# lancedb/lance

Hardware: AMD Instinct MI355X
Metric: QPS @ recall@10 (SIFT-1M IVF_PQ nlist=256 M=16) + index-build sec (higher is better)
Workload: dtype f32; 1 GPU; SIFT-1M-like 1Mx128 f32, IVF_PQ nlist=256 M=16 nbits=8, build+search on MI355X; n=1000000, d=128, nlist=256, m=16, k=10, nprobes=10, refine_factor=10, parallelism=single

## Files before the change

lance_amd/csrc/build.hip:

```cpp
#include <vector>

#include <hip/hip_fp16.h>

#include "common.h"
#include "exact.cuh"
#include <cstdlib>

#include "index.h"
#include "kernels.h"

#pragma clang fp contract(off)

namespace lh {

template <bool F16>
__global__ __launch_bounds__(256) void normalize_kernel(const float *__restrict__ x, int64_t n, int d, float *__restrict__ out) {
  const int64_t r = (int64_t)blockIdx.x * 256 + threadIdx.x;
  if (r >= n) return;
  const float *v = x + r * d;
  float acc = 0.0f;
  for (int i = 0; i < d; ++i) {
    float p = v[i] * v[i];
    if (F16) p = __half2float(__float2half_rn(p));
    acc = acc + p;
// ... 210 lines not shown
  return LANCE_HIP_OK;
}

}

using namespace lh;

lance_hip_index::~lance_hip_index() {
  (void)hipSetDevice(device);
  if (centroids) (void)hipFree(centroids);
  if (codebook) (void)hipFree(codebook);
  if (cb_mean) (void)hipFree(cb_mean);
  if (pt) {
    if (pt->g) (void)hipFree(pt->g);
    if (pt->cen_t) (void)hipFree(pt->cen_t);
    if (pt->row_beta) (void)hipFree(pt->row_beta);
    if (pt->beta_min) (void)hipFree(pt->beta_min);
    if (pt->beta_abs) (void)hipFree(pt->beta_abs);
    if (pt->beta_mean) (void)hipFree(pt->beta_mean);
    delete pt;
  }
  if (cq) {
    if (cq->cpl) (void)hipFree(cq->cpl);
    if (cq->maxbits) (void)hipFree(cq->maxbits);
    delete cq;
  }
  if (ms) {
    if (ms->cbh) (void)hipFree(ms->cbh);
    if (ms->cbn2) (void)hipFree(ms->cbn2);
    if (ms->row_cn2) (void)hipFree(ms->row_cn2);
    if (ms->cmaxp) (void)hipFree(ms->cmaxp);
    delete ms;
  }
  if (part_offsets) (void)hipFree(part_offsets);
  if (codes) (void)hipFree(codes);
  if (row_ids) (void)hipFree(row_ids);
  if (vectors) (void)hipFree(vectors);
  if (flat_items) (void)hipFree(flat_items);
  if (raw_u8) (void)hipFree(raw_u8);
  if (rq_rot_t) (void)hipFree(rq_rot_t);
}

static int encode_finish(lance_hip_ctx *ctx, uint64_t n, uint32_t nlist, const float *dists, const uint32_t *part_ids, double *loss_out_host) {
  LH_CHECK_HIP(hipGetLastError());
  if (loss_out_host) {
    std::vector<float> dh(n);
// ... 324 lines not shown
```

lance_amd/csrc/index.h:

```cpp
#pragma once
#include <atomic>
#include <cstdint>
#include <mutex>
#include <vector>

struct int2_host { int x, y; };

inline uint64_t lance_hip_next_index_serial() {
  static std::atomic<uint64_t> next{1};
  return next.fetch_add(1, std::memory_order_relaxed);
}

struct lance_hip_index {
  uint64_t serial = lance_hip_next_index_serial();
  bool ephemeral = false;
  int device = 0;
  int metric = 0;
  int dtype = 0;
  uint32_t d = 0, nlist = 0, m = 0, nbits = 8;
  uint64_t n = 0;
  float *centroids = nullptr;
  float *codebook = nullptr;
  bool model_finite = true;
  float *cb_mean = nullptr;
  struct PtConst {
    float *g = nullptr;
    float *cen_t = nullptr;
    float *row_beta = nullptr;
    float *beta_min = nullptr;
    float *beta_abs = nullptr;
    float *beta_mean = nullptr;
  } *pt = nullptr;
  struct MsConst {
    bool usable = false;
    float sigma = 1.0f;
    void *cbh = nullptr;
    float *cbn2 = nullptr;
    float *row_cn2 = nullptr;
    float cmax = 0.0f;
    float cmax_full = 0.0f;
    float *cmaxp = nullptr;
    uint32_t sum_rs = 0, max_rs = 0;
  } *ms = nullptr;
  struct CqConst {
    uint16_t *cpl = nullptr;
    uint32_t *maxbits = nullptr;
  } *cq = nullptr;
  std::mutex lazy_mu;
  uint32_t *part_offsets = nullptr;
  std::vector<uint32_t> part_offsets_h;
  uint8_t *codes = nullptr;
  uint64_t *row_ids = nullptr;
  int2_host *flat_items = nullptr;
  uint32_t n_flat_items = 0;
  float *vectors = nullptr;
  const void *raw = nullptr;
  uint64_t n_raw = 0;
  uint8_t *raw_u8 = nullptr;
  uint64_t raw_gen = 0;
  int raw_compact_state = 0;
  bool sq = false;
  double sq_lo = 0.0, sq_hi = 0.0;
  uint32_t sq_nlist = 0, sq_ld = 0;
  const uint32_t *sq_xx = nullptr;
  bool rq = false;
  uint32_t rq_nlist = 0, rq_cb = 0;
  float *rq_rot_t = nullptr;
  const float *rq_add = nullptr;
// ... 6 lines not shown
```

lance_amd/csrc/kernels.h:

```cpp
#pragma once
#include <stdint.h>

#include "common.h"
#include "search_plan.h"

namespace lh {

struct PairwiseArgs {
  const void *x_native = nullptr;
  int x_dtype = 0;
  const float *x = nullptr;
  bool lanes32 = false;
  int64_t n = 0;
  int64_t ldx = 0;
  int x_batch_off = 0;
  const float *cent = nullptr;
  int k = 0;
  int64_t cent_batch_stride = 0;
  const float *bias = nullptr;
  int64_t bias_batch_stride = 0;
  uint32_t *ids = nullptr;
  float *dists = nullptr;
  int64_t out_batch_stride = 0;
  uint8_t *codes = nullptr;
// ... 97 lines not shown
int widen_into(lance_hip_ctx *ctx, int dtype, const void *p, size_t count, float *dst);
int from_f32(lance_hip_ctx *ctx, int dtype, const float *src, void *dst, size_t count);
int launch_residual(lance_hip_ctx *ctx, const float *x, int64_t n, int d, const float *cent, const uint32_t *part_ids, float *out, bool f16);


int ivfpq_scan_merge_pm(lance_hip_ctx *ctx, const lance_hip_index *ix, const IvfpqPlan &plan, const float *qs, uint32_t nq, const uint32_t *probes,
                        uint32_t nprobes, uint32_t keff, uint32_t k, bool do_refine, uint64_t *ids, float *dists,
                        uint64_t *cand_rid, uint32_t *cand_cnt, uint32_t *flags, const uint32_t *allow);
int find_partitions_f32(lance_hip_ctx *ctx, int metric, const float *qf, uint32_t nq, uint32_t d, const float *cf, uint32_t nlist,
                        uint32_t nprobes, uint32_t *part_ids, float *dists, bool lanes32);
struct PairLists {
  const uint64_t *row_ids;
  int nprobes, k;
  uint32_t *pkey, *ppos;
  uint32_t *pcnt, *pamb;
  uint32_t *flags;
  uint32_t *n_replay;
};
int sq_merge_pairs(lance_hip_ctx *ctx, const PairLists &pl, uint32_t nq, uint64_t *ids, float *dists, const char *timer);
bool flat_small_supported(int metric, int dtype, uint32_t d, uint32_t nq, uint32_t k, uint64_t n);
int flat_topk_small(lance_hip_ctx *ctx, int metric, int dtype, const void *x, const uint64_t *row_ids, uint64_t n, uint32_t d, const float *q,
                    uint32_t nq, uint32_t k, uint64_t *ids, float *dists, bool *done);
bool coarse_mfma_supported(int metric, int d, uint32_t nq, uint32_t nlist, uint32_t nprobes, bool lanes32, const float *q, const float *cent);
int find_partitions_mfma(lance_hip_ctx *ctx, int metric, const float *q, uint32_t nq, int d, const float *cent, uint32_t nlist, uint32_t nprobes,
                         float *matrix, uint32_t *part_ids, float *dists, const uint16_t *cpl_ready = nullptr, const uint32_t *maxbits_ready = nullptr);
int launch_normalize(lance_hip_ctx *ctx, const float *x, int64_t n, int d, float *out, bool f16);
int launch_normalize_planes(lance_hip_ctx *ctx, const float *x, int64_t n, int d, float *out, bool f16, uint16_t *plane16, int dp, float *n2);

int qscan_index_constants(lance_hip_ctx *ctx, lance_hip_index *ix);
int index_alloc_like_pq(lance_hip_ctx *ctx, const lance_hip_index *src, lance_hip_index **out);
constexpr int QSCAN_SEG_CAP = 256;
struct SelectOut;
int qscan_classb_to_rescan(lance_hip_ctx *ctx, const uint32_t *tbound, uint32_t nq, uint32_t nprobes, uint32_t *seg_cnt, uint32_t *qovf);
int qscan_nearest_keys(lance_hip_ctx *ctx, const uint32_t *probes, uint32_t nq, uint32_t nprobes, uint32_t *keys, uint32_t nb = 1);
int qscan_group(lance_hip_ctx *ctx, const uint32_t *probes, uint32_t nq, uint32_t nprobes, int nlist, const uint32_t *tglobal,
                uint32_t *keys, uint32_t *tbound, uint32_t *pair_starts, uint32_t *pair_idx, uint32_t *item_start4, int4 *desc4,
                uint32_t max_items4, int G = 4, int dot = 0);
int qbound_launch(lance_hip_ctx *ctx, const lance_hip_index *ix, const float *qs, uint32_t nq, uint32_t keff, const uint32_t *pair_starts0,
                  const uint32_t *pair_idx0, uint32_t *item_start, int4 *desc, uint32_t max_items, uint32_t *tglobal, const uint32_t *allow);
int qscan_launch(lance_hip_ctx *ctx, const lance_hip_index *ix, const float *qs, uint32_t nq, uint32_t nprobes, const uint32_t *pair_idx,
                 const uint32_t *item_start4, const int4 *desc4, uint32_t max_items4, const uint32_t *tbound, uint32_t *seg_cnt,
                 uint32_t *seg_pos, uint32_t *qovf, const uint32_t *allow, const uint32_t *probes, const IvfpqPlan &plan);
int qbound_pt_launch(lance_hip_ctx *ctx, const lance_hip_index *ix, const float *qs, uint32_t nq, uint32_t nprobes, uint32_t keff,
                     const uint32_t *probes, const uint32_t *pair_starts0, const uint32_t *pair_idx0, uint32_t *item_start, int4 *desc,
                     uint32_t max_items, uint32_t *tglobal, const uint32_t *allow);
int qmerge_launch(lance_hip_ctx *ctx, const lance_hip_index *ix, const float *qs, uint32_t nq, const uint32_t *probes, uint32_t nprobes,
                  const uint32_t *tbound, uint32_t *tglobal, const uint32_t *seg_cnt, const uint32_t *seg_pos, const uint32_t *qovf,
                  uint32_t *pool_key, uint32_t *pool_pos, uint32_t *pool_cnt, int pool_cap, const SelectOut &o, const uint32_t *allow,
// ... 15 lines not shown
```

lance_amd/csrc/mfma_assign.hip:

```cpp
#include <algorithm>
#include <cstdlib>
#include <cstring>

#include <hip/hip_fp16.h>

#include "common.h"
#include "exact.cuh"
#include "kernels.h"
#include "ma_common.cuh"

#pragma clang fp contract(off)

namespace lh {

__global__ __launch_bounds__(64) void ma_prep_kernel(const float *__restrict__ cent, int k, int d, int dp, const float *__restrict__ bias,
                                                     uint16_t *__restrict__ chi, uint16_t *__restrict__ clo, float *__restrict__ cn,
                                                     uint32_t *__restrict__ maxbits ,
                                                     const uint8_t *__restrict__ active) {
  if (active && !active[0]) return;
  const int c = blockIdx.x;
  float s = 0.0f;
  for (int e = threadIdx.x; e < dp; e += 64) {
    const float v = e < d ? cent[(int64_t)c * d + e] : 0.0f;
    const uint32_t hb = bf16_rne_bits(v);
// ... 1021 lines not shown
      for (int dd = k2 >> 1; dd > 0; dd >>= 1) {
        if (dd >= 64) {
          const unsigned long long a = v2[0], b = v2[1];
          if (a > b) { v2[0] = b; v2[1] = a; }
        } else {
#pragma unroll
          for (int jr = 0; jr < 2; ++jr) {
            const int e = jr * 64 + lane;
            const unsigned long long o = __shfl_xor(v2[jr], dd, 64);
            const bool up = (e & k2) == 0, lower = (lane & dd) == 0;
            v2[jr] = (lower == up) ? (v2[jr] < o ? v2[jr] : o) : (v2[jr] > o ? v2[jr] : o);
          }
        }
      }
    }
    if (base + 64 >= cnt) break;
  }
  if (lane < nprobes) {
    part_ids[(int64_t)qi * nprobes + lane] = (uint32_t)v2[0];
    if (dists) dists[(int64_t)qi * nprobes + lane] = key_to_float((uint32_t)(v2[0] >> 32));
  }
}

bool coarse_mfma_supported(int metric, int d, uint32_t nq, uint32_t nlist, uint32_t nprobes, bool lanes32, const float *q, const float *cent) {
  static const char *env = getenv("LANCE_HIP_MFMA_COARSE");
  static const bool off = env && env[0] == '0', force = env && env[0] == '1';
  if (off || lanes32 || (metric != METRIC_L2 && metric != METRIC_DOT)) return false;
  if (nprobes == 0 || nprobes > 64 || nprobes > nlist) return false;
  if ((reinterpret_cast<uintptr_t>(q) | reinterpret_cast<uintptr_t>(cent)) & 15) return false;
  if (d <= 128) { if (d % 16 != 0 || d < 16 || nlist < 32) return false; }
  else if (d > 4096 || nlist < 64 || d % 4 != 0) return false;
  if (force) return true;
  if (d > 128) return (uint64_t)nq * nlist >= (1ull << 23);
  return (uint64_t)nq * nlist * (uint64_t)d >= (1ull << 27);
}

template <int KS>
static void coarse_launch_narrow(lance_hip_ctx *ctx, const MaArgs &a, int metric, dim3 grid) {
  constexpr int D = KS * 16;
  const size_t lds_x = (size_t)MA_ROWS * (D + 4) * 4;
  const size_t lds_c = (size_t)2 * 2 * MA_CT * (D + 8) * 2 + (size_t)2 * 2 * MA_CT * 4;
  const size_t lds = std::max(lds_x, lds_c);
  if (a.gkey) {
    if (metric == METRIC_DOT) hipLaunchKernelGGL((ma_top3_kernel<KS, METRIC_DOT, float, 2>), grid, dim3(256), lds, ctx->stream, a);
    else hipLaunchKernelGGL((ma_top3_kernel<KS, METRIC_L2, float, 2>), grid, dim3(256), lds, ctx->stream, a);
    return;
  }
  if (metric == METRIC_DOT) hipLaunchKernelGGL((ma_top3_kernel<KS, METRIC_DOT, float, 1>), grid, dim3(256), lds, ctx->stream, a);
  else hipLaunchKernelGGL((ma_top3_kernel<KS, METRIC_L2, float, 1>), grid, dim3(256), lds, ctx->stream, a);
}

static int coarse_groups_from() {
  static const int v = getenv("LANCE_HIP_COARSE_GROUPS") ? atoi(getenv("LANCE_HIP_COARSE_GROUPS")) : 1024;
  return v;
}
bool coarse_groups_shape(int d, uint32_t nlist) {
  static const bool ma = getenv("LANCE_HIP_COARSE_GROUPS_MA") != nullptr;
  return !ma && d <= 128 && d % 16 == 0 && coarse_groups_from() > 0 && nlist >= (uint32_t)std::max(coarse_groups_from(), 256);
}

int find_partitions_mfma(lance_hip_ctx *ctx, int metric, const float *q, uint32_t nq, int d, const float *cent, uint32_t nlist, uint32_t nprobes,
                         float *matrix, uint32_t *part_ids, float *dists, const uint16_t *cpl_ready, const uint32_t *maxbits_ready) {
  const bool wide = d > 128;
  const int dp = wide ? (d + MW_KC - 1) / MW_KC * MW_KC : d;
  const size_t kd = (size_t)nlist * dp;
  uint16_t *chi = ctx->scratch_t<uint16_t>("cq.chi", kd), *clo = ctx->scratch_t<uint16_t>("cq.clo", kd);
  float *cn = ctx->scratch_t<float>("cq.cn", (size_t)nlist);
  uint32_t *maxbits = ctx->scratch_t<uint32_t>("cq.maxbits", 4);
  float *e2 = ctx->scratch_t<float>("cq.e2", (size_t)nq);
  if (!chi || !clo || !cn || !maxbits || !e2) return LANCE_HIP_ENOMEM;
  const int groups_from = coarse_groups_from();
  const bool groups = !wide && groups_from > 0 && nlist >= (uint32_t)std::max(groups_from, 256);
  const int ng = groups ? (int)cdiv(nlist, MA_CT) * 4 : 0;
  float *gkey = nullptr, *gsec = nullptr;
  if (groups) {
    gkey = ctx->scratch_t<float>("cq.gkey", (size_t)nq * 2 * ng);
    gsec = gkey;
    if (!gkey) return LANCE_HIP_ENOMEM;
  }
  LH_CHECK_HIP(lh::memset_async(maxbits, 0, 16, ctx->stream));
  static const bool groups_ma = getenv("LANCE_HIP_COARSE_GROUPS_MA") != nullptr;
  if (groups && !groups_ma) {
    ScopedTimer t(ctx, "dist_matrix");
    LH_TRY(launch_xform_sweep_groups(ctx, metric, q, nq, d, cent, nlist, maxbits, gkey, ng, e2, cpl_ready, maxbits_ready));
  } else {
// ... 69 lines not shown
```

lance_amd/csrc/search.hip:

```cpp
#include <algorithm>
#include <cstdlib>
#include <string>
#include <vector>

#include "common.h"
#include "exact.cuh"
#include "index.h"
#include "kernels.h"
#include "search_common.cuh"

#pragma clang fp contract(off)

namespace lh {

#ifndef LH_SCAN_CAP
#define LH_SCAN_CAP 1024
#endif
#ifndef LH_SCAN_ROUND
#define LH_SCAN_ROUND 512
#endif
#ifndef LH_LUT_BATCH
#define LH_LUT_BATCH 4
#endif
constexpr int SCAN_CAP = LH_SCAN_CAP;
// ... 880 lines not shown
      const f4 v = x[i * 4 + p];
      uint32_t pk = 0;
#pragma unroll
      for (int e = 0; e < 4; ++e) {
        const uint32_t b = (v[e] >= 0.0f && v[e] < 256.0f) ? (uint32_t)v[e] : 0u;
        ok = ok && (float)b == v[e];
        pk |= b << (8 * e);
      }
      w[p] = pk;
    }
    out[i] = make_uint4(w[0], w[1], w[2], w[3]);
  }
  if (__any(!ok) && (threadIdx.x & 63) == 0) atomicOr(bad, 1u);
}

static bool raw_compact_enabled() {
  static const bool off = getenv("LANCE_HIP_NO_RAW_COMPACT") != nullptr;
  return !off;
}
int coarse_planes_prepare(lance_hip_ctx *ctx, const lance_hip_index *ix_c, int scan_metric) {
  lance_hip_index *ix = const_cast<lance_hip_index *>(ix_c);
  std::lock_guard<std::mutex> lk(ix->lazy_mu);
  if (ix->cq || ctx->capturing) return LANCE_HIP_OK;
  auto *cq = new lance_hip_index::CqConst();
  bool ok = hipMalloc(reinterpret_cast<void **>(&cq->cpl), xform_coarse_planes_elems(ix->nlist, (int)ix->d) * 2) == hipSuccess;
  ok = ok && hipMalloc(reinterpret_cast<void **>(&cq->maxbits), 16) == hipSuccess;
  auto drop = [&]() { if (cq->cpl) (void)hipFree(cq->cpl); if (cq->maxbits) (void)hipFree(cq->maxbits); delete cq; };
  if (!ok) { (void)hipGetLastError(); drop(); return LANCE_HIP_OK; }
  if (lh::memset_async(cq->maxbits, 0, 16, ctx->stream) != hipSuccess ||
      xform_coarse_planes(ctx, scan_metric, ix->centroids, ix->nlist, (int)ix->d, cq->cpl, cq->maxbits) != LANCE_HIP_OK ||
      hipStreamSynchronize(ctx->stream) != hipSuccess) {
    drop();
    set_error("find_partitions: building the centroid planes of the index failed");
    return LANCE_HIP_ERUNTIME;
  }
  ix->cq = cq;
  return LANCE_HIP_OK;
}

const uint8_t *raw_compact_prepare(lance_hip_ctx *ctx, const lance_hip_index *ix_c) {
  lance_hip_index *ix = const_cast<lance_hip_index *>(ix_c);
  if (!raw_compact_enabled() || ix->dtype != LANCE_HIP_F32 || !ix->raw || ix->n_raw == 0 || (ix->d & 15) != 0 ||
      (ix->metric != LANCE_HIP_L2 && ix->metric != LANCE_HIP_DOT) || (reinterpret_cast<uintptr_t>(ix->raw) & 15) != 0)
    return nullptr;
  std::lock_guard<std::mutex> lk(ix->lazy_mu);
  if (ix->raw_compact_state != 0) return ix->raw_compact_state > 0 ? ix->raw_u8 : nullptr;
  if (ctx->capturing) return nullptr;
  const uint64_t bytes = ix->n_raw * (uint64_t)ix->d;
  uint8_t *buf = nullptr;
  uint32_t *bad = ctx->scratch_t<uint32_t>("raw.compact_flag", 1);
  if (!bad || hipMalloc(reinterpret_cast<void **>(&buf), bytes) != hipSuccess) {
    (void)hipGetLastError();
    ix->raw_compact_state = -1;
// ... 406 lines not shown

  uint32_t *flags = ctx->scratch_t<uint32_t>("search.flags", (size_t)nq + 1);
  if (!flags) return LANCE_HIP_ENOMEM;
  LH_CHECK_HIP(lh::memset_async(flags, 0, ((size_t)nq + 1) * 4, ctx->stream));
  uint32_t *n_fallback = flags + nq;
  ctx->last_replay_counter = n_fallback;
  if (flags_out) *flags_out = flags;
  if (nq == 0) return LANCE_HIP_OK;

  float *qn = ix->metric == LANCE_HIP_COSINE ? ctx->scratch_t<float>("search.qnorm", (size_t)nq * d) : nullptr;
  if (ix->metric == LANCE_HIP_COSINE && !qn) return LANCE_HIP_ENOMEM;
  const float *qs = qn ? qn : q;
  PlanBatch pb;
  pb.nq = nq; pb.nprobes = nprobes; pb.keff = keff; pb.has_range = has_range != 0;
  IvfpqPlan plan = plan_ivfpq_search(plan_index(ix, qs), pb, plan_switches_from_env());
  if (plan.wants_ms_constants) {
    LH_REQUIRE(!ctx->capturing, "search: the index's matrix-core constants would have to be built during a graph capture");
    LH_TRY(mscan_prepare(ctx, const_cast<lance_hip_index *>(ix)));
    plan = plan_ivfpq_search(plan_index(ix, qs), pb, plan_switches_from_env());
  }
  static const bool q_stats = getenv("LANCE_HIP_Q_STATS") != nullptr;
  if (q_stats && plan.route != ROUTE_QUANTISED) fprintf(stderr, "[plan] nq=%u nprobes=%u keff=%u route %d: %s\n", nq, nprobes, keff, (int)plan.route, plan.why);
  if (qn) LH_TRY(launch_normalize(ctx, q, (int64_t)nq, d, qn, ix->dtype == LANCE_HIP_F16));
  float *matrix = ctx->scratch_t<float>("search.matrix", (size_t)nq * nlist);
  uint32_t *probes = ctx->scratch_t<uint32_t>("search.probes", (size_t)nq * nprobes);
  if (!matrix || !probes) return LANCE_HIP_ENOMEM;
  const bool coarse_l32 = ix->dtype == LANCE_HIP_F16 && scan_metric == LANCE_HIP_DOT && d > 16;
  if (coarse_mfma_supported(scan_metric, d, nq, (uint32_t)nlist, nprobes, coarse_l32, qs, ix->centroids)) {
    const uint16_t *cpl = nullptr;
    const uint32_t *cmb = nullptr;
    if (coarse_groups_shape(d, (uint32_t)nlist)) {
      LH_TRY(coarse_planes_prepare(ctx, ix, scan_metric));
      if (ix->cq) { cpl = ix->cq->cpl; cmb = ix->cq->maxbits; }
    }
    LH_TRY(find_partitions_mfma(ctx, scan_metric, qs, nq, d, ix->centroids, (uint32_t)nlist, nprobes, matrix, probes, nullptr, cpl, cmb));
  } else {
    PairwiseArgs pa;
    pa.x = qs; pa.n = nq; pa.ldx = d; pa.cent = ix->centroids; pa.k = nlist; pa.matrix = matrix;
    pa.lanes32 = coarse_l32;
    LH_TRY(launch_dist_matrix(ctx, pa, d, scan_metric, 1));
    ScopedTimer t(ctx, "select_probes");
    launch_select_probes(ctx, matrix, nlist, (int)nprobes, (int)nq, probes, nullptr);
  }
  uint64_t *cand_rid = nullptr;
  uint32_t *cand_cnt = nullptr;
  if (do_refine) {
    cand_rid = ctx->scratch_t<uint64_t>("search.cand_rid", (size_t)nq * keff);
    cand_cnt = ctx->scratch_t<uint32_t>("search.cand_cnt", nq);
    if (!cand_rid || !cand_cnt) return LANCE_HIP_ENOMEM;
  }
  const bool fast = plan.route != ROUTE_EXACT_ONLY;
  const bool use_pm = plan.route == ROUTE_PAIR_SCAN || plan.route == ROUTE_QUANTISED;
  int nsplit = 1;
  if (nq < (uint32_t)(2 * ctx->num_cus)) {
    nsplit = (int)std::min<uint64_t>({8ull, (uint64_t)nprobes, cdiv(2ull * ctx->num_cus, nq)});
    if (nsplit < 1) nsplit = 1;
  }
  const size_t nblk = (size_t)nq * nsplit;
// ... 61 lines not shown
    const int dpad = (d + 3) & ~3;
    const size_t lds = (size_t)dpad * 4 + (size_t)m * 256 * 4 + (size_t)keff * 12 + ((size_t)keff + 1) * 8 + 64 * 4 + 16 +
                       16 + (size_t)std::max<uint32_t>(200, keff) * 4 + (size_t)m * 16 + 16;
    LH_REQUIRE(lds <= 160 * 1024, "search: exact kernel does not fit in LDS (m=%d, k*refine=%u)", m, keff);
    ScopedTimer t(ctx, "ivfpq_exact");
    if (ix->nbits == 4) {
      if (scan_metric == LANCE_HIP_DOT) hipLaunchKernelGGL((ivfpq_exact_kernel<METRIC_DOT, 4>), dim3(nq), dim3(64), lds, ctx->stream, ea);
      else hipLaunchKernelGGL((ivfpq_exact_kernel<METRIC_L2, 4>), dim3(nq), dim3(64), lds, ctx->stream, ea);
    } else {
      if (scan_metric == LANCE_HIP_DOT) hipLaunchKernelGGL((ivfpq_exact_kernel<METRIC_DOT, 8>), dim3(nq), dim3(64), lds, ctx->stream, ea);
      else hipLaunchKernelGGL((ivfpq_exact_kernel<METRIC_L2, 8>), dim3(nq), dim3(64), lds, ctx->stream, ea);
    }
  }
  if (do_refine) LH_TRY(launch_refine(ctx, ix, q, nq, d, cand_rid, cand_cnt, keff, k, ids, dists, flags, nullptr));
  LH_CHECK_HIP(hipGetLastError());
  return LANCE_HIP_OK;
}

int find_partitions_f32(lance_hip_ctx *ctx, int metric, const float *qf, uint32_t nq, uint32_t d, const float *cf, uint32_t nlist,
                        uint32_t nprobes, uint32_t *part_ids, float *dists, bool lanes32) {
  if (nprobes > nlist) nprobes = nlist;
  LH_REQUIRE(nlist <= 8192 || nprobes <= 2048, "find_partitions: nprobes=%u > 2048 with more than 8192 partitions is not supported", nprobes);
  if (nq == 0 || nprobes == 0) return LANCE_HIP_OK;
  float *matrix = ctx->scratch_t<float>("search.matrix", (size_t)nq * nlist);
  if (!matrix) return LANCE_HIP_ENOMEM;
  const int km = metric == LANCE_HIP_COSINE ? LANCE_HIP_L2 : metric;
  if (coarse_mfma_supported(km, (int)d, nq, nlist, nprobes, lanes32, qf, cf)) {
    LH_TRY(find_partitions_mfma(ctx, km, qf, nq, (int)d, cf, nlist, nprobes, matrix, part_ids, dists));
  } else {
    PairwiseArgs pa;
    pa.x = qf; pa.n = nq; pa.ldx = d;
    pa.cent = cf; pa.k = (int)nlist; pa.matrix = matrix;
    pa.lanes32 = lanes32;
    LH_TRY(launch_dist_matrix(ctx, pa, (int)d, km, 1));
    launch_select_probes(ctx, matrix, (int)nlist, (int)nprobes, (int)nq, part_ids, dists);
  }
  LH_CHECK_HIP(hipGetLastError());
  LH_CHECK_HIP(hipStreamSynchronize(ctx->stream));
  return LANCE_HIP_OK;
}

static int check_flags(lance_hip_ctx *ctx, const uint32_t *flags, uint32_t nq) {
  std::vector<uint32_t> fh(nq);
  LH_CHECK_HIP(hipMemcpyAsync(fh.data(), flags, (size_t)nq * 4, hipMemcpyDeviceToHost, ctx->stream));
  LH_CHECK_HIP(hipStreamSynchronize(ctx->stream));
  uint32_t n_over = 0, n_amb = 0, n_bad = 0;
  for (uint32_t i = 0; i < nq; ++i) { n_over += (fh[i] & FLAG_OVERFLOW) ? 1 : 0; n_amb += (fh[i] & FLAG_AMBIGUOUS) ? 1 : 0; n_bad += (fh[i] & FLAG_BADROW) ? 1 : 0; }
  if (n_bad) {
    set_error("search: refine met row ids beyond the %s raw vectors given to lance_hip_index_set_raw (%u queries): the raw array must be "
              "indexed by the stored row ids", "attached", n_bad);
    return LANCE_HIP_EINVAL;
  }
  if (n_over || n_amb) {
    set_error("search: internal error, %u overflow / %u ambiguous queries were not resolved by the exact kernel", n_over, n_amb);
    return LANCE_HIP_ERUNTIME;
  }
  return LANCE_HIP_OK;
}

}

using namespace lh;

extern "C" {

int lance_hip_index_prewarm(lance_hip_ctx *ctx, lance_hip_index *idx) {
  lh::CtxLock _ctx_lock(ctx);
  LH_REQUIRE(ctx && idx, "index_prewarm: NULL argument");
  LH_CHECK_HIP(hipSetDevice(ctx->device));
  if (idx->m > 0 && !plan_index_ms_refusal(plan_index(idx, nullptr), plan_switches_from_env())) LH_TRY(mscan_prepare(ctx, idx));
  if (coarse_groups_shape((int)idx->d, idx->nlist) && (reinterpret_cast<uintptr_t>(idx->centroids) & 15) == 0)
    LH_TRY(coarse_planes_prepare(ctx, idx, idx->metric == LANCE_HIP_COSINE ? LANCE_HIP_L2 : idx->metric));
  (void)raw_compact_prepare(ctx, idx);
  LH_CHECK_HIP(hipStreamSynchronize(ctx->stream));
  return LANCE_HIP_OK;
}

int lance_hip_find_partitions(lance_hip_ctx *ctx, int dtype, int metric, const void *q, uint32_t nq, uint32_t d,
                              const void *centroids, uint32_t nlist, uint32_t nprobes, uint32_t *part_ids, float *dists) {
  lh::CtxLock _ctx_lock(ctx);
  LH_REQUIRE(ctx && q && centroids && part_ids, "find_partitions: NULL argument");
  LH_TRY(check_dtype(dtype, "find_partitions"));
  LH_REQUIRE(nlist > 0 && nlist <= 65536, "find_partitions: nlist=%u not supported in this version (1..65536)", nlist);
  LH_CHECK_HIP(hipSetDevice(ctx->device));
  const float *qf, *cf;
  LH_TRY(as_f32(ctx, dtype, q, (size_t)nq * d, "f16.q", &qf));
  LH_TRY(as_f32(ctx, model_dtype(dtype), centroids, (size_t)nlist * d, "f16.cent", &cf));
  return find_partitions_f32(ctx, metric, qf, nq, d, cf, nlist, nprobes, part_ids, dists, dtype == LANCE_HIP_F16 && metric == LANCE_HIP_DOT && d > 16);
}

int lance_hip_ivfpq_search_async(lance_hip_ctx *ctx, const lance_hip_index *idx, const void *q, uint32_t nq, uint32_t k,
                                 uint32_t nprobes, uint32_t refine_factor, uint64_t *ids, float *dists) {
  lh::CtxLock _ctx_lock(ctx);
  LH_REQUIRE(ctx && idx && (nq == 0 || (q && ids && dists)), "search: NULL argument");
// ... 166 lines not shown
```

Baseline: 25.38 million queries/s.

## Fuse coarse centroid distance GEMM with top-nprobes selection in one kernel

Adds a fused coarse-quantizer kernel. It computes query-centroid distances with split-bf16 MFMA (hi/lo planes) into LDS, then picks the probe candidates within an error bound, rescored exactly in fp32, all in the same kernel. This removes the nq x nlist distance matrix written to global memory and the separate select_probes launch. Centroid hi/lo planes and norms are precomputed and cached per index. Rows with too many or too few candidates, or NaN, fall back to an exact per-row scan, which adds complexity and can be slow when many rows take that path.

```diff
diff --git a/lance_amd/csrc/build.hip b/lance_amd/csrc/build.hip
--- a/lance_amd/csrc/build.hip
+++ b/lance_amd/csrc/build.hip
@@ -256,6 +256,7 @@
   }
   if (cq) {
     if (cq->cpl) (void)hipFree(cq->cpl);
+    if (cq->chi) (void)hipFree(cq->chi);
     if (cq->maxbits) (void)hipFree(cq->maxbits);
     delete cq;
   }
diff --git a/lance_amd/csrc/index.h b/lance_amd/csrc/index.h
--- a/lance_amd/csrc/index.h
+++ b/lance_amd/csrc/index.h
@@ -44,6 +44,8 @@
   } *ms = nullptr;
   struct CqConst {
     uint16_t *cpl = nullptr;
+    uint16_t *chi = nullptr, *clo = nullptr;
+    float *cn = nullptr;
     uint32_t *maxbits = nullptr;
   } *cq = nullptr;
   std::mutex lazy_mu;
diff --git a/lance_amd/csrc/kernels.h b/lance_amd/csrc/kernels.h
--- a/lance_amd/csrc/kernels.h
+++ b/lance_amd/csrc/kernels.h
@@ -143,8 +143,17 @@
 int flat_topk_small(lance_hip_ctx *ctx, int metric, int dtype, const void *x, const uint64_t *row_ids, uint64_t n, uint32_t d, const float *q,
                     uint32_t nq, uint32_t k, uint64_t *ids, float *dists, bool *done);
 bool coarse_mfma_supported(int metric, int d, uint32_t nq, uint32_t nlist, uint32_t nprobes, bool lanes32, const float *q, const float *cent);
+struct CoarseFusedConst {
+  const uint16_t *chi, *clo;
+  const float *cn;
+  const uint32_t *maxbits;
+};
+bool coarse_fused_shape(int d, uint32_t nlist);
+size_t coarse_fused_cn_elems(uint32_t nlist);
+int coarse_fused_planes(lance_hip_ctx *ctx, const float *cent, uint32_t nlist, int d, uint16_t *chi, uint16_t *clo, float *cn, uint32_t *maxbits );
 int find_partitions_mfma(lance_hip_ctx *ctx, int metric, const float *q, uint32_t nq, int d, const float *cent, uint32_t nlist, uint32_t nprobes,
-                         float *matrix, uint32_t *part_ids, float *dists, const uint16_t *cpl_ready = nullptr, const uint32_t *maxbits_ready = nullptr);
+                         float *matrix, uint32_t *part_ids, float *dists, const uint16_t *cpl_ready = nullptr, const uint32_t *maxbits_ready = nullptr,
+                         const CoarseFusedConst *fused_ready = nullptr);
 int launch_normalize(lance_hip_ctx *ctx, const float *x, int64_t n, int d, float *out, bool f16);
 int launch_normalize_planes(lance_hip_ctx *ctx, const float *x, int64_t n, int d, float *out, bool f16, uint16_t *plane16, int dp, float *n2);
 
diff --git a/lance_amd/csrc/mfma_assign.hip b/lance_amd/csrc/mfma_assign.hip
--- a/lance_amd/csrc/mfma_assign.hip
+++ b/lance_amd/csrc/mfma_assign.hip
@@ -1067,6 +1067,259 @@
   }
 }
 
+constexpr int CF_ROWS = 32;
+constexpr int CF_WAVES = 8;
+constexpr uint32_t CF_MAX_LISTS = 960;
+
+static size_t coarse_fused_lds(int d, uint32_t nlist) {
+  const size_t n64 = (size_t)cdiv(nlist, MA_CT) * MA_CT;
+  const size_t planes = (size_t)2 * CF_ROWS * (d + 8) * 2, cands = (size_t)CF_WAVES * CS_CAP * 12;
+  return (size_t)CF_ROWS * (d + 4) * 4 + std::max(planes, cands) + (size_t)CF_ROWS * (n64 + 4) * 4;
+}
+
+template <int CTRL, int ROW_MASK, bool SUM>
+__device__ __forceinline__ float cf_dpp_step(float v) {
+  const float ident = SUM ? 0.0f : v;
+  const float o = __builtin_bit_cast(float, __builtin_amdgcn_update_dpp(__builtin_bit_cast(int, ident), __builtin_bit_cast(int, v), CTRL, ROW_MASK, 0xF, false));
+  return SUM ? v + o : fminf(v, o);
+}
+template <bool SUM>
+__device__ __forceinline__ float cf_wave_reduce(float v) {
+  v = cf_dpp_step<0xB1, 0xF, SUM>(v);
+  v = cf_dpp_step<0x4E, 0xF, SUM>(v);
+  v = cf_dpp_step<0x141, 0xF, SUM>(v);
+  v = cf_dpp_step<0x140, 0xF, SUM>(v);
+  v = cf_dpp_step<0x142, 0xA, SUM>(v);
+  v = cf_dpp_step<0x143, 0xC, SUM>(v);
+  return __builtin_bit_cast(float, __builtin_amdgcn_readlane(__builtin_bit_cast(int, v), 63));
+}
+
+template <int KS, int METRIC>
+__global__ __launch_bounds__(64 * CF_WAVES, 4) void coarse_fused_kernel(const float *__restrict__ q, int nq, const uint16_t *__restrict__ chi,
+                                                                       const uint16_t *__restrict__ clo, const float *__restrict__ cn ,
+                                                                       const uint32_t *__restrict__ maxbits, const float *__restrict__ cent, int nlist,
+                                                                       int nprobes, uint32_t *__restrict__ part_ids, float *__restrict__ dists,
+                                                                       uint32_t *__restrict__ n_exact_rows) {
+  extern __shared__ __attribute__((aligned(16))) char smem[];
+  constexpr int D = KS * 16;
+  constexpr int XS = D + 4;
+  constexpr int CS = D + 8;
+  constexpr size_t PLANES = (size_t)2 * CF_ROWS * CS * 2, CANDS = (size_t)CF_WAVES * CS_CAP * 12;
+  const int n64 = (nlist + MA_CT - 1) / MA_CT * MA_CT;
+  const int SP = n64 + 4;
+  float *xs = reinterpret_cast<float *>(smem);
+  uint16_t *xh = reinterpret_cast<uint16_t *>(xs + CF_ROWS * XS), *xl = xh + CF_ROWS * CS;
+  unsigned long long *ck_all = reinterpret_cast<unsigned long long *>(xh);
+  uint32_t *cl_all = reinterpret_cast<uint32_t *>(ck_all + CF_WAVES * CS_CAP);
+  float *sur = reinterpret_cast<float *>(smem + (size_t)CF_ROWS * XS * 4 + (PLANES > CANDS ? PLANES : CANDS));
+  const int lane = threadIdx.x & 63, wave = threadIdx.x >> 6, grp = lane >> 4;
+  const int j = lane & 31, g = lane >> 5;
+  const int64_t row0 = (int64_t)blockIdx.x * CF_ROWS;
+
+  if ((int)threadIdx.x < CF_ROWS * (D / 8)) {
+    const int r = (int)threadIdx.x / (D / 8), c8 = (int)threadIdx.x - r * (D / 8);
+    f4 a = {0.0f, 0.0f, 0.0f, 0.0f}, b = a;
+    if (row0 + r < nq) { a = load4(q + (row0 + r) * D + 8 * c8); b = load4(q + (row0 + r) * D + 8 * c8 + 4); }
+    *reinterpret_cast<f4 *>(&xs[r * XS + 8 * c8]) = a;
+    *reinterpret_cast<f4 *>(&xs[r * XS + 8 * c8 + 4]) = b;
+    const float v[8] = {a.x, a.y, a.z, a.w, b.x, b.y, b.z, b.w};
+    bf16x8 h, l;
+#pragma unroll
+    for (int e = 0; e < 8; ++e) {
+      const uint32_t hb = bf16_rne_bits(v[e]);
+      const uint32_t lb = bf16_rne_bits(v[e] - bf16_bits_to_float(hb));
+      h[e] = (short)hb; l[e] = (short)lb;
+    }
+    *reinterpret_cast<bf16x8 *>(xh + r * CS + 8 * c8) = h;
+    *reinterpret_cast<bf16x8 *>(xl + r * CS + 8 * c8) = l;
+  }
+  __syncthreads();
+
+  const int nblocks = n64 / 32;
+  for (int blk = wave; blk < nblocks; blk += CF_WAVES) {
+    const int c0 = blk * 32;
+    const int ca = min(c0 + j, nlist - 1);
+    const uint16_t *ha = chi + (int64_t)ca * D + g * 8, *la = clo + (int64_t)ca * D + g * 8;
+    const uint16_t *bh = xh + j * CS + g * 8, *bl = xl + j * CS + g * 8;
+    bf16x8 ah[KS], al[KS];
+#pragma unroll
+    for (int s = 0; s < KS; ++s) {
+      ah[s] = *reinterpret_cast<const bf16x8 *>(ha + s * 16);
+      al[s] = *reinterpret_cast<const bf16x8 *>(la + s * 16);
+    }
+    f32x16 acc;
+#pragma unroll
+    for (int v = 0; v < 16; ++v) acc[v] = 0.0f;
+#pragma unroll
+    for (int s = 0; s < KS; ++s) {
+      const bf16x8 qh = *reinterpret_cast<const bf16x8 *>(bh + s * 16);
+      const bf16x8 ql = *reinterpret_cast<const bf16x8 *>(bl + s * 16);
+      acc = __builtin_amdgcn_mfma_f32_32x32x16_bf16(ah[s], qh, acc, 0, 0, 0);
+      acc = __builtin_amdgcn_mfma_f32_32x32x16_bf16(ah[s], ql, acc, 0, 0, 0);
+      acc = __builtin_amdgcn_mfma_f32_32x32x16_bf16(al[s], qh, acc, 0, 0, 0);
+    }
+    float *srow = sur + (size_t)j * SP;
+#pragma unroll
+    for (int vq = 0; vq < 4; ++vq) {
+      const int ib = c0 + 8 * vq + 4 * g;
+      const f4 cn4 = *reinterpret_cast<const f4 *>(cn + ib);
+      float o[4];
+#pragma unroll
+      for (int e = 0; e < 4; ++e) {
+        const float dot = acc[vq * 4 + e];
+        float v = METRIC == METRIC_DOT ? -dot : __builtin_fmaf(-2.0f, dot, cn4[e]);
+        if (ib + e >= nlist) v = INFINITY;
+        o[e] = v;
+      }
+      *reinterpret_cast<f4 *>(srow + ib) = f4{o[0], o[1], o[2], o[3]};
+    }
+  }
+  __syncthreads();
+
+  unsigned long long *ck = ck_all + wave * CS_CAP;
+  uint32_t *cl = cl_all + wave * CS_CAP;
+  const float cmax2 = __uint_as_float(maxbits[0]);
+  for (int r = wave; r < CF_ROWS; r += CF_WAVES) {
+    const int64_t qi = row0 + r;
+    if (qi >= nq) break;
+    float *row = sur + (size_t)r * SP;
+    const float *wrow = xs + r * XS;
+    float xn2 = 0.0f;
+    for (int e = lane; e < D; e += 64) xn2 += wrow[e] * wrow[e];
+    xn2 = cf_wave_reduce<true>(xn2);
+    const float E2 = 2.0f * 0.0001220703125f * (xn2 + cmax2) + (METRIC == METRIC_DOT ? 4.7683716e-7f : 0.0f);
+    bool bad = !(E2 < INFINITY) || !(E2 > 7.888609052210118e-31f);
+    float m0 = INFINITY, m1 = INFINITY, m2 = INFINITY, m3 = INFINITY;
+    for (int base = 0; base < n64; base += 256) {
+      float v4[4];
+#pragma unroll
+      for (int u = 0; u < 4; ++u) { const int i = base + 64 * u + lane; v4[u] = i < n64 ? row[i] : INFINITY; }
+#pragma unroll
+      for (int u = 0; u < 4; ++u) {
+        const float v = v4[u];
+        bad |= v != v;
+        if (v < m3) {
+          if (v < m2) {
+            m3 = m2;
+            if (v < m1) {
+              m2 = m1;
+              if (v < m0) { m1 = m0; m0 = v; } else m1 = v;
+            } else m2 = v;
+          } else m3 = v;
+        }
+      }
+    }
+    bad = __any(bad);
+    uint32_t cnt = 0;
+    if (!bad) {
+      float t0 = INFINITY;
+      for (int pr = 0; pr < nprobes; ++pr) {
+        t0 = cf_wave_reduce<false>(m0);
+        if (!(t0 < INFINITY)) break;
+        const unsigned long long holders = __ballot(m0 == t0);
+        if (lane == __ffsll((long long)holders) - 1) { m0 = m1; m1 = m2; m2 = m3; m3 = INFINITY; }
+      }
+      const float thr = t0 + E2;
+      for (int base = 0; base < nlist; base += 256) {
+        float v4[4];
+#pragma unroll
+        for (int u = 0; u < 4; ++u) { const int i = base + 64 * u + lane; v4[u] = i < nlist ? row[i] : INFINITY; }
+#pragma unroll
+        for (int u = 0; u < 4; ++u) {
+          const int i = base + 64 * u + lane;
+          const bool take = i < nlist && v4[u] <= thr;
+          const unsigned long long mask = __ballot(take);
+          if (take) {
+            const uint32_t pos = cnt + (uint32_t)__popcll(mask & ((1ull << lane) - 1ull));
+            if (pos < (uint32_t)CS_CAP) cl[pos] = (uint32_t)i;
+          }
+          cnt += (uint32_t)__popcll(mask);
+        }
+      }
+      if (cnt > (uint32_t)CS_CAP || cnt < (uint32_t)nprobes) bad = true;
+    }
+    __builtin_amdgcn_wave_barrier();
+    if (bad) {
+      if (lane == 0 && n_exact_rows) atomicAdd(n_exact_rows, 1u);
+      for (int c0 = 0; c0 < nlist; c0 += 4) {
+        const int c = c0 + grp;
+        float v = 0.0f;
+        if (c < nlist) v = cs_group_distance<METRIC>(wrow, cent + (int64_t)c * D, D, lane);
+        else (void)cs_group_distance<METRIC>(wrow, cent, D, lane);
+        if (c < nlist && (lane & 15) == 0) row[c] = v;
+      }
+      __builtin_amdgcn_wave_barrier();
+      __threadfence_block();
+      unsigned long long last = 0ull;
+      bool have_last = false;
+      for (int pr = 0; pr < nprobes; ++pr) {
+        unsigned long long best = ~0ull;
+        for (int i = lane; i < nlist; i += 64) {
+          const unsigned long long kk = ((unsigned long long)order_key(row[i]) << 32) | (uint32_t)i;
+          if ((!have_last || kk > last) && kk < best) best = kk;
+        }
+#pragma unroll
+        for (int o = 32; o > 0; o >>= 1) { const unsigned long long ob = __shfl_xor(best, o, 64); best = ob < best ? ob : best; }
+        if (lane == 0) {
+          part_ids[qi * nprobes + pr] = (uint32_t)best;
+          if (dists) dists[qi * nprobes + pr] = key_to_float((uint32_t)(best >> 32));
+        }
+        last = best; have_last = true;
+      }
+      continue;
+    }
+    for (uint32_t c0 = 0; c0 < cnt; c0 += 16) {
+      uint32_t cc[4];
+      float dv[4];
+#pragma unroll
+      for (int u = 0; u < 4; ++u) { const uint32_t ci = c0 + 4 * u + (uint32_t)grp; cc[u] = ci < cnt ? cl[ci] : cl[0]; }
+#pragma unroll
+      for (int u = 0; u < 4; ++u) dv[u] = cs_group_distance<METRIC>(wrow, cent + (int64_t)cc[u] * D, D, lane);
+#pragma unroll
+      for (int u = 0; u < 4; ++u) {
+        const uint32_t ci = c0 + 4 * u + (uint32_t)grp;
+        if (ci < cnt && (lane & 15) == 0) ck[ci] = ((unsigned long long)order_key(dv[u]) << 32) | cc[u];
+      }
+    }
+    __builtin_amdgcn_wave_barrier();
+    const unsigned long long k0 = (uint32_t)lane < cnt ? ck[lane] : ~0ull, k1 = 64u + (uint32_t)lane < cnt ? ck[64 + lane] : ~0ull;
+    uint32_t rank0 = 0, rank1 = 0;
+    for (uint32_t i = 0; i < cnt; i += 4) {
+      unsigned long long o[4];
+#pragma unroll
+      for (uint32_t u = 0; u < 4; ++u) o[u] = i + u < cnt ? ck[i + u] : ~0ull;
+#pragma unroll
+      for (uint32_t u = 0; u < 4; ++u) {
+        rank0 += o[u] < k0 ? 1u : 0u;
+        rank1 += o[u] < k1 ? 1u : 0u;
+      }
+    }
+    if ((uint32_t)lane < cnt && rank0 < (uint32_t)nprobes) {
+      part_ids[qi * nprobes + rank0] = (uint32_t)k0;
+      if (dists) dists[qi * nprobes + rank0] = key_to_float((uint32_t)(k0 >> 32));
+    }
+    if (64u + (uint32_t)lane < cnt && rank1 < (uint32_t)nprobes) {
+      part_ids[qi * nprobes + rank1] = (uint32_t)k1;
+      if (dists) dists[qi * nprobes + rank1] = key_to_float((uint32_t)(k1 >> 32));
+    }
+    __builtin_amdgcn_wave_barrier();
+  }
+}
+
+template <int KS>
+static void coarse_launch_fused(lance_hip_ctx *ctx, int metric, const float *q, uint32_t nq, const uint16_t *chi, const uint16_t *clo, const float *cn,
+                                const uint32_t *maxbits, const float *cent, uint32_t nlist, uint32_t nprobes, uint32_t *part_ids, float *dists,
+                                uint32_t *n_exact_rows) {
+  const size_t lds = coarse_fused_lds(KS * 16, nlist);
+  const dim3 grid((unsigned)cdiv(nq, CF_ROWS));
+  if (metric == METRIC_DOT)
+    hipLaunchKernelGGL((coarse_fused_kernel<KS, METRIC_DOT>), grid, dim3(64 * CF_WAVES), lds, ctx->stream, q, (int)nq, chi, clo, cn, maxbits, cent, (int)nlist,
+                       (int)nprobes, part_ids, dists, n_exact_rows);
+  else
+    hipLaunchKernelGGL((coarse_fused_kernel<KS, METRIC_L2>), grid, dim3(64 * CF_WAVES), lds, ctx->stream, q, (int)nq, chi, clo, cn, maxbits, cent, (int)nlist,
+                       (int)nprobes, part_ids, dists, n_exact_rows);
+}
+
 bool coarse_mfma_supported(int metric, int d, uint32_t nq, uint32_t nlist, uint32_t nprobes, bool lanes32, const float *q, const float *cent) {
   static const char *env = getenv("LANCE_HIP_MFMA_COARSE");
   static const bool off = env && env[0] == '0', force = env && env[0] == '1';
@@ -1104,8 +1357,66 @@
   return !ma && d <= 128 && d % 16 == 0 && coarse_groups_from() > 0 && nlist >= (uint32_t)std::max(coarse_groups_from(), 256);
 }
 
+bool coarse_fused_shape(int d, uint32_t nlist) {
+  static const bool off = getenv("LANCE_HIP_NO_COARSE_FUSED") != nullptr && getenv("LANCE_HIP_NO_COARSE_FUSED")[0] == '1';
+  return !off && d >= 16 && d <= 128 && d % 16 == 0 && nlist >= 32 && nlist <= CF_MAX_LISTS && !coarse_groups_shape(d, nlist) &&
+         coarse_fused_lds(d, nlist) <= (size_t)160 * 1024;
+}
+size_t coarse_fused_cn_elems(uint32_t nlist) { return (size_t)cdiv(nlist, MA_CT) * MA_CT; }
+int coarse_fused_planes(lance_hip_ctx *ctx, const float *cent, uint32_t nlist, int d, uint16_t *chi, uint16_t *clo, float *cn, uint32_t *maxbits) {
+  hipLaunchKernelGGL(ma_prep_kernel, dim3(nlist), dim3(64), 0, ctx->stream, cent, (int)nlist, d, d, nullptr, chi, clo, cn, maxbits, nullptr);
+  LH_CHECK_HIP(hipGetLastError());
+  return LANCE_HIP_OK;
+}
+
+static int find_partitions_fused(lance_hip_ctx *ctx, int metric, const float *q, uint32_t nq, int d, const float *cent, uint32_t nlist, uint32_t nprobes,
+                                 uint32_t *part_ids, float *dists, const CoarseFusedConst *ready) {
+  uint32_t *maxbits = ctx->scratch_t<uint32_t>("cq.maxbits", 4);
+  if (!maxbits) return LANCE_HIP_ENOMEM;
+  static const bool stats = getenv("LANCE_HIP_COARSE_STATS") != nullptr;
+  const uint16_t *chi, *clo;
+  const float *cn;
+  const uint32_t *mb;
+  ScopedTimer t(ctx, "select_probes");
+  ctx->count_stage("coarse_fused");
+  if (ready) {
+    chi = ready->chi; clo = ready->clo; cn = ready->cn; mb = ready->maxbits;
+    if (stats) LH_CHECK_HIP(lh::memset_async(maxbits, 0, 16, ctx->stream));
+  } else {
+    uint16_t *h = ctx->scratch_t<uint16_t>("cq.chi", (size_t)nlist * d), *l = ctx->scratch_t<uint16_t>("cq.clo", (size_t)nlist * d);
+    float *n = ctx->scratch_t<float>("cq.cn", coarse_fused_cn_elems(nlist));
+    if (!h || !l || !n) return LANCE_HIP_ENOMEM;
+    ctx->count_stage("coarse_fused_prep");
+    LH_CHECK_HIP(lh::memset_async(maxbits, 0, 16, ctx->stream));
+    LH_TRY(coarse_fused_planes(ctx, cent, nlist, d, h, l, n, maxbits));
+    chi = h; clo = l; cn = n; mb = maxbits;
+  }
+  switch (d / 16) {
+    case 1: coarse_launch_fused<1>(ctx, metric, q, nq, chi, clo, cn, mb, cent, nlist, nprobes, part_ids, dists, maxbits + 2); break;
+    case 2: coarse_launch_fused<2>(ctx, metric, q, nq, chi, clo, cn, mb, cent, nlist, nprobes, part_ids, dists, maxbits + 2); break;
+    case 3: coarse_launch_fused<3>(ctx, metric, q, nq, chi, clo, cn, mb, cent, nlist, nprobes, part_ids, dists, maxbits + 2); break;
+    case 4: coarse_launch_fused<4>(ctx, metric, q, nq, chi, clo, cn, mb, cent, nlist, nprobes, part_ids, dists, maxbits + 2); break;
+    case 5: coarse_launch_fused<5>(ctx, metric, q, nq, chi, clo, cn, mb, cent, nlist, nprobes, part_ids, dists, maxbits + 2); break;
+    case 6: coarse_launch_fused<6>(ctx, metric, q, nq, chi, clo, cn, mb, cent, nlist, nprobes, part_ids, dists, maxbits + 2); break;
+    case 7: coarse_launch_fused<7>(ctx, metric, q, nq, chi, clo, cn, mb, cent, nlist, nprobes, part_ids, dists, maxbits + 2); break;
+    case 8: coarse_launch_fused<8>(ctx, metric, q, nq, chi, clo, cn, mb, cent, nlist, nprobes, part_ids, dists, maxbits + 2); break;
+    default: return LANCE_HIP_EINVAL;
+  }
+  LH_CHECK_HIP(hipGetLastError());
+  if (stats && !ctx->capturing) {
+    uint32_t h[4];
+    LH_CHECK_HIP(hipMemcpyAsync(h, maxbits, 16, hipMemcpyDeviceToHost, ctx->stream));
+    LH_CHECK_HIP(hipStreamSynchronize(ctx->stream));
+    fprintf(stderr, "[coarse] nq=%u nlist=%u nprobes=%u fused=1: %u queries took the exact path\n", nq, nlist, nprobes, h[2]);
+  }
+  return LANCE_HIP_OK;
+}
+
 int find_partitions_mfma(lance_hip_ctx *ctx, int metric, const float *q, uint32_t nq, int d, const float *cent, uint32_t nlist, uint32_t nprobes,
-                         float *matrix, uint32_t *part_ids, float *dists, const uint16_t *cpl_ready, const uint32_t *maxbits_ready) {
+                         float *matrix, uint32_t *part_ids, float *dists, const uint16_t *cpl_ready, const uint32_t *maxbits_ready,
+                         const CoarseFusedConst *fused_ready) {
+  if (coarse_fused_shape(d, nlist)) return find_partitions_fused(ctx, metric, q, nq, d, cent, nlist, nprobes, part_ids, dists, fused_ready);
+  LH_REQUIRE(matrix, "find_partitions: no matrix scratch for a shape the fused kernel does not serve");
   const bool wide = d > 128;
   const int dp = wide ? (d + MW_KC - 1) / MW_KC * MW_KC : d;
   const size_t kd = (size_t)nlist * dp;
diff --git a/lance_amd/csrc/search.hip b/lance_amd/csrc/search.hip
--- a/lance_amd/csrc/search.hip
+++ b/lance_amd/csrc/search.hip
@@ -926,13 +926,22 @@
   lance_hip_index *ix = const_cast<lance_hip_index *>(ix_c);
   std::lock_guard<std::mutex> lk(ix->lazy_mu);
   if (ix->cq || ctx->capturing) return LANCE_HIP_OK;
+  const bool fused = coarse_fused_shape((int)ix->d, ix->nlist);
   auto *cq = new lance_hip_index::CqConst();
-  bool ok = hipMalloc(reinterpret_cast<void **>(&cq->cpl), xform_coarse_planes_elems(ix->nlist, (int)ix->d) * 2) == hipSuccess;
+  const size_t kd = (size_t)ix->nlist * ix->d;
+  bool ok;
+  if (fused) {
+    ok = hipMalloc(reinterpret_cast<void **>(&cq->chi), kd * 2 * 2 + coarse_fused_cn_elems(ix->nlist) * 4) == hipSuccess;
+    if (ok) { cq->clo = cq->chi + kd; cq->cn = reinterpret_cast<float *>(cq->clo + kd); }
+  } else {
+    ok = hipMalloc(reinterpret_cast<void **>(&cq->cpl), xform_coarse_planes_elems(ix->nlist, (int)ix->d) * 2) == hipSuccess;
+  }
   ok = ok && hipMalloc(reinterpret_cast<void **>(&cq->maxbits), 16) == hipSuccess;
-  auto drop = [&]() { if (cq->cpl) (void)hipFree(cq->cpl); if (cq->maxbits) (void)hipFree(cq->maxbits); delete cq; };
+  auto drop = [&]() { if (cq->cpl) (void)hipFree(cq->cpl); if (cq->chi) (void)hipFree(cq->chi); if (cq->maxbits) (void)hipFree(cq->maxbits); delete cq; };
   if (!ok) { (void)hipGetLastError(); drop(); return LANCE_HIP_OK; }
   if (lh::memset_async(cq->maxbits, 0, 16, ctx->stream) != hipSuccess ||
-      xform_coarse_planes(ctx, scan_metric, ix->centroids, ix->nlist, (int)ix->d, cq->cpl, cq->maxbits) != LANCE_HIP_OK ||
+      (fused ? coarse_fused_planes(ctx, ix->centroids, ix->nlist, (int)ix->d, cq->chi, cq->clo, cq->cn, cq->maxbits)
+             : xform_coarse_planes(ctx, scan_metric, ix->centroids, ix->nlist, (int)ix->d, cq->cpl, cq->maxbits)) != LANCE_HIP_OK ||
       hipStreamSynchronize(ctx->stream) != hipSuccess) {
     drop();
     set_error("find_partitions: building the centroid planes of the index failed");
@@ -1385,18 +1394,24 @@
   static const bool q_stats = getenv("LANCE_HIP_Q_STATS") != nullptr;
   if (q_stats && plan.route != ROUTE_QUANTISED) fprintf(stderr, "[plan] nq=%u nprobes=%u keff=%u route %d: %s\n", nq, nprobes, keff, (int)plan.route, plan.why);
   if (qn) LH_TRY(launch_normalize(ctx, q, (int64_t)nq, d, qn, ix->dtype == LANCE_HIP_F16));
-  float *matrix = ctx->scratch_t<float>("search.matrix", (size_t)nq * nlist);
+  const bool coarse_l32 = ix->dtype == LANCE_HIP_F16 && scan_metric == LANCE_HIP_DOT && d > 16;
+  const bool coarse_mfma = coarse_mfma_supported(scan_metric, d, nq, (uint32_t)nlist, nprobes, coarse_l32, qs, ix->centroids);
+  const bool coarse_fused = coarse_mfma && coarse_fused_shape(d, (uint32_t)nlist);
+  float *matrix = coarse_fused ? nullptr : ctx->scratch_t<float>("search.matrix", (size_t)nq * nlist);
   uint32_t *probes = ctx->scratch_t<uint32_t>("search.probes", (size_t)nq * nprobes);
-  if (!matrix || !probes) return LANCE_HIP_ENOMEM;
-  const bool coarse_l32 = ix->dtype == LANCE_HIP_F16 && scan_metric == LANCE_HIP_DOT && d > 16;
-  if (coarse_mfma_supported(scan_metric, d, nq, (uint32_t)nlist, nprobes, coarse_l32, qs, ix->centroids)) {
+  if ((!matrix && !coarse_fused) || !probes) return LANCE_HIP_ENOMEM;
+  if (coarse_mfma) {
     const uint16_t *cpl = nullptr;
     const uint32_t *cmb = nullptr;
-    if (coarse_groups_shape(d, (uint32_t)nlist)) {
+    CoarseFusedConst cf{};
+    bool have_cf = false;
+    if (coarse_fused || coarse_groups_shape(d, (uint32_t)nlist)) {
       LH_TRY(coarse_planes_prepare(ctx, ix, scan_metric));
-      if (ix->cq) { cpl = ix->cq->cpl; cmb = ix->cq->maxbits; }
-    }
-    LH_TRY(find_partitions_mfma(ctx, scan_metric, qs, nq, d, ix->centroids, (uint32_t)nlist, nprobes, matrix, probes, nullptr, cpl, cmb));
+      if (ix->cq && coarse_fused) { cf = CoarseFusedConst{ix->cq->chi, ix->cq->clo, ix->cq->cn, ix->cq->maxbits}; have_cf = true; }
+      else if (ix->cq) { cpl = ix->cq->cpl; cmb = ix->cq->maxbits; }
+    }
+    LH_TRY(find_partitions_mfma(ctx, scan_metric, qs, nq, d, ix->centroids, (uint32_t)nlist, nprobes, matrix, probes, nullptr, cpl, cmb,
+                                have_cf ? &cf : nullptr));
   } else {
     PairwiseArgs pa;
     pa.x = qs; pa.n = nq; pa.ldx = d; pa.cent = ix->centroids; pa.k = nlist; pa.matrix = matrix;
@@ -1504,10 +1519,12 @@
   if (nprobes > nlist) nprobes = nlist;
   LH_REQUIRE(nlist <= 8192 || nprobes <= 2048, "find_partitions: nprobes=%u > 2048 with more than 8192 partitions is not supported", nprobes);
   if (nq == 0 || nprobes == 0) return LANCE_HIP_OK;
-  float *matrix = ctx->scratch_t<float>("search.matrix", (size_t)nq * nlist);
-  if (!matrix) return LANCE_HIP_ENOMEM;
   const int km = metric == LANCE_HIP_COSINE ? LANCE_HIP_L2 : metric;
-  if (coarse_mfma_supported(km, (int)d, nq, nlist, nprobes, lanes32, qf, cf)) {
+  const bool mfma = coarse_mfma_supported(km, (int)d, nq, nlist, nprobes, lanes32, qf, cf);
+  const bool fused = mfma && coarse_fused_shape((int)d, nlist);
+  float *matrix = fused ? nullptr : ctx->scratch_t<float>("search.matrix", (size_t)nq * nlist);
+  if (!matrix && !fused) return LANCE_HIP_ENOMEM;
+  if (mfma) {
     LH_TRY(find_partitions_mfma(ctx, km, qf, nq, (int)d, cf, nlist, nprobes, matrix, part_ids, dists));
   } else {
     PairwiseArgs pa;
@@ -1551,7 +1568,7 @@
   LH_REQUIRE(ctx && idx, "index_prewarm: NULL argument");
   LH_CHECK_HIP(hipSetDevice(ctx->device));
   if (idx->m > 0 && !plan_index_ms_refusal(plan_index(idx, nullptr), plan_switches_from_env())) LH_TRY(mscan_prepare(ctx, idx));
-  if (coarse_groups_shape((int)idx->d, idx->nlist) && (reinterpret_cast<uintptr_t>(idx->centroids) & 15) == 0)
+  if ((coarse_groups_shape((int)idx->d, idx->nlist) || coarse_fused_shape((int)idx->d, idx->nlist)) && (reinterpret_cast<uintptr_t>(idx->centroids) & 15) == 0)
     LH_TRY(coarse_planes_prepare(ctx, idx, idx->metric == LANCE_HIP_COSINE ? LANCE_HIP_L2 : idx->metric));
   (void)raw_compact_prepare(ctx, idx);
   LH_CHECK_HIP(hipStreamSynchronize(ctx->stream));
```

Result: faster. 27.11 million queries/s, median of 6 (+6.8%).
